# jneem/nnnoiseless

Hardware: AMD Instinct MI355X
Metric: 480-sample frames/sec (whole node) at N concurrent streams (higher is better)
Workload: dtype f32; 1 GPU; configs[2]: 65536 concurrent streams on one GPU, built-in weights.rnn, GRU as batched MFMA GEMM, synthetic 48 kHz sine+noise, 48 frame(s) per stream per step; parity=oracle pinned by the reference's golden pair (built-in model), model=built-in weights.rnn, boundary_format=f32 planar (process_frame's own), streams_per_gpu=65536, streams_total=65536, inputs_ready=True, schedule=stages, lanes=2, parallelism=streams sharded x1, one process per GPU, no data-path collective

## Files before the change

### nnnoiseless_amd/csrc/nnn_synth.hip

```cpp
#pragma once

namespace nnn {

__device__ __forceinline__ float interp_gain(const float *g, int k, const float *bin_frac, const unsigned char *bin_band)
{
    if (k >= 400) return 0.0f;
    int i = bin_band[k];
    float frac = bin_frac[bsk(k)];
    return fmaf(frac, g[i + 1], (1.0f - frac) * g[i]);
}
__device__ __forceinline__ void interp_gain2(const float *ga, const float *gb, int k, const float *bin_frac, const unsigned char *bin_band,
                                             float &ra, float &rb)
{
    ra = 0.0f;
    rb = 0.0f;
    if (k >= 400) return;
    const int i = bin_band[k];
    const float frac = bin_frac[bsk(k)], om = 1.0f - frac;
    ra = fmaf(frac, ga[i + 1], om * ga[i]);
    rb = fmaf(frac, gb[i + 1], om * gb[i]);
}

struct BinConst { int band[8]; float frac[8]; };
template <bool SMV_IO, bool PLAIN = false>
__device__ __forceinline__ void synth_frame(const Buffers &b, const StepParams *sp, int f, int tile, int sl, int s, int lane, const FftLds &t, float2 *A,
                                         float *r, float2 (&Xr)[8], const float2 (&Pk)[8], float b_ex, float b_ep, float b_xp, float b_graw,
                                         float b_g, float vadv, bool live, float *sm, float4 (&smq)[2], const BinConst *bc = nullptr)
{
    if (SMV_IO) {
#pragma unroll
        for (int u = 0; u < 2; u++) smq[u] = lane + 64 * u < FRAME / 4 ? ((const float4 *)sm)[lane + 64 * u] : make_float4(0.0f, 0.0f, 0.0f, 0.0f);
    }
    float *ebuf = (float *)A, *r2 = r + NB, *gg = r + 2 * NB;
    float *vad_out = sp->vad;
    const int fmt = PLAIN ? (int)PCM_F32 : sp->fmt;
    const int ch = PLAIN ? 1 : sp->channels, grp = s / ch, elem = pcm_elem_bytes(fmt), sstride = ch * elem;
    char *o = sp->out + (long long)grp * sp->group_stride + (long long)(s - grp * ch) * elem;
    const bool store = s < b.S && !sp->discard;
    int bmask = 1 << NB;
    if (live) {
        const bool up = b_xp > b_graw;
        const int mask = (int)(wave_ballot(up && lane < NB) & ((1ull << NB) - 1));
        if (lane < NB) {
            float v;
            if (up) v = 1.0f;
            else {
                float exp_sq = b_xp * b_xp, g_sq = b_graw * b_graw;
                v = exp_sq * (1.0f - g_sq) / (0.001f + g_sq * (1.0f - exp_sq));
            }
            v = sqrtf(fminf(fmaxf(v, 0.0f), 1.0f));
            v *= sqrtf(b_ex / (1e-8f + b_ep));
            r[lane] = v;
            gg[lane] = b_g;
        }
        wave_lds_sync();
        if (lane == 0) {
            NNN_TIF(b, branch, 1, f, tile, sl)[0] = mask;
            bmask = mask;
        }
#pragma unroll
        for (int u = 0; u < 8; u++) {
            const int k = rfft_slot_bin(lane, u);
            if (k >= 0) {
                float2 X = Xr[u];
                const float2 P = k < 400 ? Pk[u] : make_float2(0.0f, 0.0f);
                float rf;
                if (!SMV_IO && bc) {
                    const int i = bc->band[u] < 0 ? 0 : bc->band[u];
                    const float fr = bc->frac[u];
                    rf = bc->band[u] < 0 ? 0.0f : fmaf(fr, r[i + 1], (1.0f - fr) * r[i]);
                } else rf = interp_gain(r, k, t.frac, t.band);
                X.x = fmaf(P.x, rf, X.x);
                X.y = fmaf(P.y, rf, X.y);
                Xr[u] = X;
                if (k < 400) ebuf[bsk(k)] = fmaf(X.y, X.y, X.x * X.x);
            }
        }
        wave_lds_sync();
        {
            const float *const v[1] = {ebuf};
            float ne[1];
            band_sums_par<1>(t, v, ne, lane);
            if (lane < NB) r2[lane] = sqrtf(b_ex / (1e-8f + ne[0]));
        }
        wave_lds_sync();
#pragma unroll
        for (int u = 0; u < 8; u++) {
            const int k = rfft_slot_bin(lane, u);
            if (k >= 0) {
                float rf, gf;
                if (!SMV_IO && bc) {
                    const int i = bc->band[u] < 0 ? 0 : bc->band[u];
                    const float fr = bc->frac[u], om = 1.0f - fr;
                    rf = bc->band[u] < 0 ? 0.0f : fmaf(fr, r2[i + 1], om * r2[i]);
                    gf = bc->band[u] < 0 ? 0.0f : fmaf(fr, gg[i + 1], om * gg[i]);
                } else interp_gain2(r2, gg, k, t.frac, t.band, rf, gf);
                Xr[u].x *= rf; Xr[u].y *= rf;
                Xr[u].x *= gf; Xr[u].y *= gf;
            }
        }
    } else if (lane == 0) {
        NNN_TIF(b, branch, 1, f, tile, sl)[0] = 1 << NB;
    }
    if (sp->log && s < b.S) {
        unsigned *lg = sp->log + (size_t)s * FRAME_LOG_WORDS;
        if (lane < NB) lg[2 + lane] = __float_as_uint(live ? b_g : 0.0f);
        if (lane == 0) {
            lg[0] = (unsigned)NNN_TIF(b, pitch, 1, f, tile, sl)[0];
            lg[1] = (unsigned)bmask;
        }
    }
#pragma unroll
    for (int u = 0; u < 8; u++) {
        const int k = rfft_slot_bin(lane, u);
        if (k >= 0) A[k] = Xr[u];
    }
    wave_lds_sync();
    float2 zin[8];
    {
        const int j = lane < FFT_P1 ? lane : FFT_P1 - 1;
#pragma unroll
        for (int rr = 0; rr < 8; rr++) {
            const int k = j + FFT_P1 * rr;
            float2 a = A[k], c = A[NFFT - k];
            float2 e2 = make_float2(a.x + c.x, a.y - c.y);
            float2 d = make_float2(a.x - c.x, a.y + c.y);
            float2 w = t.tw[k];
            w.y = -w.y;
            float2 o2 = cmulf(d, w);
            zin[rr] = make_float2(e2.y + o2.x, e2.x - o2.y);
        }
    }
    wave_lds_sync();
    float4 wlo[2], whi[2];
#pragma unroll
    for (int u = 0; u < 2; u++) {
        const int n = lane + 64 * u;
        const bool on = n < FRAME / 4;
        wlo[u] = on ? ((const float4 *)b.window_s)[n] : make_float4(0.0f, 0.0f, 0.0f, 0.0f);
        whi[u] = on ? ((const float4 *)b.window_s)[FRAME / 4 + n] : make_float4(0.0f, 0.0f, 0.0f, 0.0f);
    }
    fft480_regs<true, !SMV_IO>(zin, A, t.tw, lane);
    if (lane == 0 && vad_out && s < b.S) vad_out[s] = vadv;
    const bool quad_ok = ch == 1 && (((size_t)o) & (size_t)(4 * elem - 1)) == 0;
#pragma unroll
    for (int u = 0; u < 2; u++) {
        const int n = lane + 64 * u;
        if (n < FRAME / 4) {
            const float4 lo = ((const float4 *)A)[n], hi = ((const float4 *)A)[n + FRAME / 4];
            const float u0 = hi.y * whi[u].x, u1 = hi.x * whi[u].y, u2 = hi.w * whi[u].z, u3 = hi.z * whi[u].w;
            if (store) {
                const float y0 = fmaf(lo.y, wlo[u].x, smq[u].x), y1 = fmaf(lo.x, wlo[u].y, smq[u].y), y2 = fmaf(lo.w, wlo[u].z, smq[u].z),
                            y3 = fmaf(lo.z, wlo[u].w, smq[u].w);
                if (quad_ok && fmt == PCM_F32) ((float4 *)o)[n] = make_float4(y0, y1, y2, y3);
                else if (quad_ok && fmt == PCM_I16)
                    ((uint2 *)o)[n] = make_uint2((unsigned)(unsigned short)pcm_to_i16(y0) | ((unsigned)(unsigned short)pcm_to_i16(y1) << 16),
                                                 (unsigned)(unsigned short)pcm_to_i16(y2) | ((unsigned)(unsigned short)pcm_to_i16(y3) << 16));
                else if (quad_ok) ((float4 *)o)[n] = make_float4(pcm_to_unit(y0), pcm_to_unit(y1), pcm_to_unit(y2), pcm_to_unit(y3));
                else {
                    pcm_store(o + (long long)(4 * n) * sstride, fmt, y0);
                    pcm_store(o + (long long)(4 * n + 1) * sstride, fmt, y1);
                    pcm_store(o + (long long)(4 * n + 2) * sstride, fmt, y2);
                    pcm_store(o + (long long)(4 * n + 3) * sstride, fmt, y3);
                }
            }
            smq[u] = make_float4(u0, u1, u2, u3);
            if (SMV_IO) ((float4 *)sm)[n] = smq[u];
        }
    }
    wave_lds_sync();
}

#ifndef NNN_SYN_MINWAVES
#define NNN_SYN_MINWAVES 4
#endif
template <bool PLAIN>
__global__ void __launch_bounds__(64 * FFT_SPB, NNN_SYN_MINWAVES) k_synth(Buffers b, const StepParams *sp0, int g)
{
    __shared__ FftLds t;
    __shared__ float2 A_[FFT_SPB][NFFT_BUF];
    __shared__ float r_[FFT_SPB][3 * NB];
    const int wave = threadIdx.x >> 6;
    float2 *A = A_[wave];
    float *r = r_[wave];
    int tile, sub;
    xcd_tile_block((int)blockIdx.x, b.NT, TILE / FFT_SPB, tile, sub);
    if (tile * TILE + sub * FFT_SPB >= b.S) return;
    if (!live_any(b, tile, sub * FFT_SPB, FFT_SPB)) return;
    const int lane0 = threadIdx.x & 63, sl = sub * FFT_SPB + wave, s = tile * TILE + sl;
    int lane = lane0;
    fft_tables_load(t, b, true);
    float *sm = b.synth_mem + (size_t)s * FRAME;
    float4 smq[2];
#pragma unroll
    for (int u = 0; u < 2; u++) smq[u] = lane + 64 * u < FRAME / 4 ? ((const float4 *)sm)[lane + 64 * u] : make_float4(0.0f, 0.0f, 0.0f, 0.0f);
    __syncthreads();
    BinConst bc;
#pragma unroll
    for (int u = 0; u < 8; u++) {
        const int k = rfft_slot_bin(lane0, u);
        const bool on = k >= 0 && k < 400;
        bc.band[u] = on ? (int)t.band[on ? k : 0] : -1;
        bc.frac[u] = on ? t.frac[bsk(on ? k : 0)] : 0.0f;
    }
    const int s_out = live_stream(b, tile, sl) ? s : b.S_pad;
    for (int f = 0; f < g; f++) {
        lane = launder_v(lane0);
        const size_t fo = (size_t)b.S_pad * (size_t)f;
        const float2 *Xg = b.X + (fo + s) * FSTR, *Pg = b.P + (fo + s) * FSTR;
        const bool live = NNN_TIF(b, silence, 1, f, tile, sl)[0] == 0;
        float2 Xr[8], Pr[8];
        spectrum_load(Xg, Xr, lane);
        spectrum_load_p(Pg, Pr, lane);
        float b_ex = 0.0f, b_ep = 0.0f, b_xp = 0.0f, b_graw = 0.0f, b_g = 0.0f;
        if (lane < NB) {
            b_ex = NNN_TIF(b, ex, NB, f, tile, sl)[(size_t)lane * TILE];
            b_ep = NNN_TIF(b, ep, NB, f, tile, sl)[(size_t)lane * TILE];
            b_xp = NNN_TIF(b, exp_, NB, f, tile, sl)[(size_t)lane * TILE];
            b_graw = NNN_TIF(b, g_raw, NB, f, tile, sl)[(size_t)lane * TILE];
            b_g = NNN_TIF(b, g, NB, f, tile, sl)[(size_t)lane * TILE];
        }
        const float vadv = NNN_TIF(b, vad, 1, f, tile, sl)[0];
        synth_frame<false, PLAIN>(b, sp0 + f, f, tile, sl, s_out, lane, t, A, r, Xr, Pr, b_ex, b_ep, b_xp, b_graw, b_g, vadv, live, sm, smq, &bc);
    }
#pragma unroll
    for (int u = 0; u < 2; u++)
        if (lane0 + 64 * u < FRAME / 4) ((float4 *)sm)[lane0 + 64 * u] = smq[u];
}

#pragma clang fp contract(off)

}
```

Before: 75.05 million frames/s.

## Prefetch next frame's spectra and gains during synthesis inverse FFT

```diff
diff --git a/nnnoiseless_amd/csrc/nnn_synth.hip b/nnnoiseless_amd/csrc/nnn_synth.hip
--- a/nnnoiseless_amd/csrc/nnn_synth.hip
+++ b/nnnoiseless_amd/csrc/nnn_synth.hip
@@ -22,10 +22,12 @@
 }
 
 struct BinConst { int band[8]; float frac[8]; };
-template <bool SMV_IO, bool PLAIN = false>
+struct SynthNoHook { __device__ __forceinline__ void operator()() const {} };
+template <bool SMV_IO, bool PLAIN = false, class TRANSFORMED = SynthNoHook>
 __device__ __forceinline__ void synth_frame(const Buffers &b, const StepParams *sp, int f, int tile, int sl, int s, int lane, const FftLds &t, float2 *A,
                                          float *r, float2 (&Xr)[8], const float2 (&Pk)[8], float b_ex, float b_ep, float b_xp, float b_graw,
-                                         float b_g, float vadv, bool live, float *sm, float4 (&smq)[2], const BinConst *bc = nullptr)
+                                         float b_g, float vadv, bool live, float *sm, float4 (&smq)[2], const BinConst *bc = nullptr,
+                                         TRANSFORMED &&transformed = SynthNoHook())
 {
     if (SMV_IO) {
 #pragma unroll
@@ -141,6 +143,7 @@
         whi[u] = on ? ((const float4 *)b.window_s)[FRAME / 4 + n] : make_float4(0.0f, 0.0f, 0.0f, 0.0f);
     }
     fft480_regs<true, !SMV_IO>(zin, A, t.tw, lane);
+    transformed();
     if (lane == 0 && vad_out && s < b.S) vad_out[s] = vadv;
     const bool quad_ok = ch == 1 && (((size_t)o) & (size_t)(4 * elem - 1)) == 0;
 #pragma unroll
@@ -171,11 +174,18 @@
     wave_lds_sync();
 }
 
+__device__ __forceinline__ void vm_wait_all()
+{
+#ifdef __HIPCC__
+    __builtin_amdgcn_s_waitcnt(0x0F70);
+#endif
+}
+
 #ifndef NNN_SYN_MINWAVES
 #define NNN_SYN_MINWAVES 4
 #endif
 template <bool PLAIN>
-__global__ void __launch_bounds__(64 * FFT_SPB, NNN_SYN_MINWAVES) k_synth(Buffers b, const StepParams *sp0, int g)
+__global__ void __launch_bounds__(64 * FFT_SPB, NNN_SYN_MINWAVES) k_synth(Buffers b, const StepParams *__restrict__ sp0, int g)
 {
     __shared__ FftLds t;
     __shared__ float2 A_[FFT_SPB][NFFT_BUF];
@@ -204,24 +214,39 @@
         bc.frac[u] = on ? t.frac[bsk(on ? k : 0)] : 0.0f;
     }
     const int s_out = live_stream(b, tile, sl) ? s : b.S_pad;
+    const int sl_u = __builtin_amdgcn_readfirstlane(sl);
+    const size_t step1 = (size_t)b.S_pad, stepb = step1 * NB, stepx = step1 * FSTR;
+    size_t o1 = (size_t)tile * TILE + sl_u, ob = (size_t)tile * TILE * NB + sl_u, ox = o1 * FSTR;
+    float2 Xr[8], Pr[8];
+    float b_ex, b_ep, b_xp, b_graw, b_g, vadv;
+    int silent;
+    auto fetch = [&](int ln, bool on) {
+        silent = 0;
+        vadv = b_ex = b_ep = b_xp = b_graw = b_g = 0.0f;
+#pragma unroll
+        for (int u = 0; u < 8; u++) Xr[u] = Pr[u] = make_float2(0.0f, 0.0f);
+        if (!on) return;
+        silent = b.silence[o1];
+        if (ln < NB) {
+            b_xp = b.exp_[ob + (size_t)ln * TILE];
+            b_graw = b.g_raw[ob + (size_t)ln * TILE];
+            b_ex = b.ex[ob + (size_t)ln * TILE];
+            b_ep = b.ep[ob + (size_t)ln * TILE];
+            b_g = b.g[ob + (size_t)ln * TILE];
+        }
+        vadv = b.vad[o1];
+        spectrum_load(b.X + ox, Xr, ln);
+        spectrum_load_p(b.P + ox, Pr, ln);
+    };
+    fetch(lane0, true);
     for (int f = 0; f < g; f++) {
         lane = launder_v(lane0);
-        const size_t fo = (size_t)b.S_pad * (size_t)f;
-        const float2 *Xg = b.X + (fo + s) * FSTR, *Pg = b.P + (fo + s) * FSTR;
-        const bool live = NNN_TIF(b, silence, 1, f, tile, sl)[0] == 0;
-        float2 Xr[8], Pr[8];
-        spectrum_load(Xg, Xr, lane);
-        spectrum_load_p(Pg, Pr, lane);
-        float b_ex = 0.0f, b_ep = 0.0f, b_xp = 0.0f, b_graw = 0.0f, b_g = 0.0f;
-        if (lane < NB) {
-            b_ex = NNN_TIF(b, ex, NB, f, tile, sl)[(size_t)lane * TILE];
-            b_ep = NNN_TIF(b, ep, NB, f, tile, sl)[(size_t)lane * TILE];
-            b_xp = NNN_TIF(b, exp_, NB, f, tile, sl)[(size_t)lane * TILE];
-            b_graw = NNN_TIF(b, g_raw, NB, f, tile, sl)[(size_t)lane * TILE];
-            b_g = NNN_TIF(b, g, NB, f, tile, sl)[(size_t)lane * TILE];
-        }
-        const float vadv = NNN_TIF(b, vad, 1, f, tile, sl)[0];
-        synth_frame<false, PLAIN>(b, sp0 + f, f, tile, sl, s_out, lane, t, A, r, Xr, Pr, b_ex, b_ep, b_xp, b_graw, b_g, vadv, live, sm, smq, &bc);
+        const bool live = silent == 0;
+        synth_frame<false, PLAIN>(b, sp0 + f, f, tile, sl, s_out, lane, t, A, r, Xr, Pr, b_ex, b_ep, b_xp, b_graw, b_g, vadv, live, sm, smq, &bc, [&]() {
+            vm_wait_all();
+            o1 += step1; ob += stepb; ox += stepx;
+            fetch(lane, f + 1 < g);
+        });
     }
 #pragma unroll
     for (int u = 0; u < 2; u++)
```

Result: faster. 76.46 million frames/s (median of 6 runs) (+1.9%).
